# shanjiayao/PTT

Measured on AMD Instinct MI355X. Metric: tracklet frames/sec (hot path: PointNet++ SA stack + Point-Track-Transformer blocks), higher is better.
Workload: dtype f32

## Files before the change

include/ptt_hip.h:

```cpp
#ifndef PTT_HIP_H
#define PTT_HIP_H

#include <stddef.h>
#include <stdint.h>

#ifdef __cplusplus
extern "C" {
#endif

#define PTT_ABI_VERSION 39

enum {
    PTT_OK = 0,
    PTT_EINVAL = -1,
    PTT_EUNSUPPORTED = -2,
    PTT_ELAUNCH = -3,
    PTT_EWORKSPACE = -4
};

typedef void* ptt_stream_t;

int ptt_version(void);
const char* ptt_error_name(int code);
const char* ptt_last_error_string(void);

int ptt_fps_f32(const float* xyz, int B, int N, int npoint, int32_t* idx_out,
                ptt_stream_t stream);
int ptt_fps_ws_f32(const float* xyz, int B, int N, int npoint, int32_t* idx_out, float* workspace,
                   size_t workspace_elems, ptt_stream_t stream);

int ptt_ffps_f32(const float* xyz, const float* feat, int64_t feat_sb, int64_t feat_sc, int64_t feat_sn,
                 int B, int N, int C, int npoint, int32_t* idx_out, ptt_stream_t stream);

int ptt_gather_f32(const float* feat, const int32_t* idx, int B, int C, int N, int M,
                   float* out, ptt_stream_t stream);
int ptt_gather_grad_f32(const float* grad_out, const int32_t* idx, int B, int C, int N,
                        int M, float* grad_feat, ptt_stream_t stream);

int ptt_select_centres_f32(const float* xyz, const int32_t* idx, int B, int N, int M, float* new_xyz,
                           int64_t* idx64_out, ptt_stream_t stream);

int ptt_ball_query_f32(const float* new_xyz, const float* xyz, int B, int M, int N,
                       float radius, int nsample, int32_t* idx_out, ptt_stream_t stream);

int ptt_centres_ball_query_f32(const float* xyz, const int32_t* sel, int B, int N, int M, float radius, int nsample,
                               float* new_xyz, int64_t* idx64_out, int32_t* idx_out, ptt_stream_t stream);

int ptt_group_f32(const float* feat, const int32_t* idx, int B, int C, int N, int M,
                  int ns, float* out, ptt_stream_t stream);
int ptt_group_grad_f32(const float* grad_out, const int32_t* idx, int B, int C, int N,
                       int M, int ns, float* grad_feat, ptt_stream_t stream);

size_t ptt_scatter_add_det_workspace(int B, int N, int E);
int ptt_scatter_add_det_f32(const float* src, const int32_t* idx, int B, int C, int N, int E, float* out,
                            void* workspace, size_t workspace_bytes, ptt_stream_t stream);

int ptt_knn_f32(const float* xyz, int B, int N, int k, int32_t* idx_out,
                ptt_stream_t stream);
int ptt_knn_rel_f32(const float* xyz, int B, int N, int k, int32_t* idx_out, float* rel_out,
                    ptt_stream_t stream);

size_t ptt_packed_weight_elems(int Cout, int K);
int ptt_pack_weight_f32(const float* W, int Cout, int K, float* packed,
                        ptt_stream_t stream);
int ptt_pack_weight_rot_f32(const float* W, int Cout, int K, int rot, float* packed,
                            ptt_stream_t stream);

int ptt_linear_f32(const float* X, int rows, int K, int ldx, const float* Wpacked, int Cout,
                   const float* scale, const float* shift, int relu, const float* residual,
                   int ldr, float* out, int ldo, ptt_stream_t stream);

#define PTT_SA_MAX_LAYERS 4

typedef struct ptt_sa_layer {
    const float* Wpacked;
    const float* scale;
    const float* shift;
    int Cin;
    int Cout;
    int relu;
} ptt_sa_layer;

int ptt_rows_mlp_f32(const float* X, int rows, int K, int ldx, const ptt_sa_layer* layers, int n_layers,
                     const float* residual, int ldr, float* out, int ldo, ptt_stream_t stream);

size_t ptt_ball_query_grid_workspace(int B, int N);
int ptt_ball_query_grid_f32(const float* new_xyz, const float* xyz, int B, int M, int N, float radius, int nsample,
                            int32_t* idx_out, void* workspace, size_t workspace_bytes, ptt_stream_t stream);
int ptt_centres_ball_query_grid_f32(const float* xyz, const int32_t* sel, int B, int N, int M, float radius, int nsample,
                                    float* new_xyz, int64_t* idx64_out, int32_t* idx_out, void* workspace, size_t workspace_bytes,
                                    ptt_stream_t stream);
int ptt_fps_ball_knn_f32(const float* xyz, int B, int N, int M, float radius, int nsample, int k, int32_t* inds,
                         int64_t* inds64, float* new_xyz, int32_t* idx, int32_t* knn, float* rel, ptt_stream_t stream);
// ... 254 lines not shown
#define PTT_REF_CAMERA 0
#define PTT_REF_LIDAR 1
int ptt_box_overlap_f64(const double* gt, const double* pred, int n, int ref_coord, int dims, double* overlap, double* accuracy,
                        ptt_stream_t stream);

#define PTT_TRAIN_MAX_CANDS 1024
typedef struct ptt_train_cand {
    const float* search;
    const uint8_t* label;
    const float* first;
    const float* prev;
    const int32_t* counts;
    float reg[4];
    uint32_t index;
    uint32_t epoch;
    int32_t capacity;
    int32_t reserved;
} ptt_train_cand;

typedef struct ptt_train_batch_desc {
    float* search_points;
    float* template_points;
    float* cls_label;
    float* reg_label;
    int32_t* src_out;
    int32_t* idx_search_out;
    int32_t* idx_template_out;
    int32_t* info;
    int64_t* totals;
    int32_t B, n_cand;
    int32_t search_size, template_size;
    int32_t min_points;
    uint32_t seed_lo, seed_hi;
    int32_t reserved;
} ptt_train_batch_desc;

int ptt_train_batch_f32(const ptt_train_cand* cands_device, const ptt_train_batch_desc* desc_host, ptt_stream_t stream);

typedef struct ptt_train_aug {
    float m[4];
    float kz;
    float reserved[3];
} ptt_train_aug;

int ptt_train_batch_aug_f32(const ptt_train_cand* cands_device, const ptt_train_aug* aug_device, const ptt_train_batch_desc* desc_host,
                            ptt_stream_t stream);
int ptt_philox4x32_10(const uint32_t* counter4, const uint32_t* key2, uint32_t* out4);

size_t ptt_bn_stats_workspace(int R, int C);
int ptt_bn_stats_f32(const float* X, int R, int C, int ldx, float eps, float* mean, float* var, float* invstd,
                     void* workspace, size_t workspace_bytes, ptt_stream_t stream);
int ptt_bn_apply_f32(const float* Z, int ldz, const float* mean, const float* invstd, const float* gamma,
                     const float* beta, int R, int C, int relu, float* X, int ldx, ptt_stream_t stream);
int ptt_bn_bwd_f32(const float* G, int ldg, const float* Act, int lda, const float* Z, int ldz, const float* mean,
                   const float* invstd, const float* gamma, int R, int C, int relu, float* dZ, int ldd,
                   float* dgamma, float* dbeta, void* workspace, size_t workspace_bytes, const float* act_scale,
                   const float* act_shift, ptt_stream_t stream);
int ptt_bn_sums_f64(const float* X, int R, int C, int ldx, double* sums, void* workspace, size_t workspace_bytes,
                    ptt_stream_t stream);
int ptt_bn_finish_f64(const double* sums, int C, float eps, float* mean, float* var, float* invstd,
                      ptt_stream_t stream);
int ptt_bn_bwd_sums_f64(const float* G, int ldg, const float* Act, int lda, const float* Z, int ldz, const float* mean,
                        const float* invstd, int R, int C, double* sums, void* workspace, size_t workspace_bytes,
                        const float* act_scale, const float* act_shift, ptt_stream_t stream);
int ptt_bn_bwd_apply_f32(const float* G, int ldg, const float* Act, int lda, const float* Z, int ldz, const float* mean,
                         const float* invstd, const float* gamma, const float* sum_dy, const float* sum_dy_xhat,
                         const double* count, int R, int C, float* dZ, int ldd, const float* act_scale, const float* act_shift,
                         ptt_stream_t stream);
int ptt_pool_rows_f32(const float* X, int ldx, int G, int ns, int C, float* out, int ldo, int32_t* arg,
                      const float* act_scale, const float* act_shift, ptt_stream_t stream);
int ptt_pool_rows_bwd_f32(const float* dOut, int ldo, const int32_t* arg, int G, int ns, int C, float* dX, int ldx,
                          ptt_stream_t stream);
int ptt_pt_pair_input_f32(const float* q, const float* kf, const int32_t* knn, const float* pos, int B, int N, int k, int D,
                          float* t, ptt_stream_t stream);
int ptt_pt_attn_train_fwd_f32(const float* a, const float* vf, const int32_t* knn, const float* pos, int B, int N, int k, int D,
                              float scale, float* attn, float* res, ptt_stream_t stream);
int ptt_pt_attn_train_bwd_f32(const float* attn, const float* vf, const int32_t* knn, const float* pos, const float* dres, int B,
                              int N, int k, int D, float scale, float* da, float* dvp, ptt_stream_t stream);

int ptt_pt_pair_input_ld_f32(const float* q, int ldq, const float* kf, int ldk, const int32_t* knn, const float* pos, int B, int N,
                             int k, int D, float* t, ptt_stream_t stream);
int ptt_pt_attn_fwd_ld_f32(const float* a, const float* vf, int ldv, const int32_t* knn, const float* pos, int B, int N, int k, int D,
                           float scale, float* attn, float* res, ptt_stream_t stream);

int ptt_gather_rows_f32(const float* src, const int32_t* idx, int B, int N, int E, int C, float* out, ptt_stream_t stream);
int ptt_scatter_csr_i32(const int32_t* idx, int B, int N, int E, int32_t* order, int32_t* start, ptt_stream_t stream);
int ptt_scatter_rows_csr_f32(const float* g, const int32_t* order, const int32_t* start, int B, int N, int E, int C,
                             float* out, ptt_stream_t stream);
int ptt_rows_gemm_pool_supported(int rows, int K, int N, int ldx, int ns);
int ptt_rows_gemm_pool_f32(const float* X, int rows, int K, int ldx, const float* in_scale, const float* in_shift,
                           const float* Wpacked, int N, float* out, int ldo, double* stats, size_t stats_elems, int ns,
                           float* pmax, float* pmin, int32_t* amax, int32_t* amin, ptt_stream_t stream);
int ptt_pool_select_f32(const float* pmax, const float* pmin, const int32_t* amax, const int32_t* amin, const float* act_scale,
                        const float* act_shift, int G, int C, float* out, int32_t* arg, ptt_stream_t stream);
size_t ptt_colsum_workspace(int R, int C);
int ptt_colsum_f32(const float* X, int R, int C, int ldx, float* out, void* workspace, size_t workspace_bytes, ptt_stream_t stream);
size_t ptt_linear_wgrad_workspace(int R, int Cout, int Cin);
int ptt_linear_wgrad_f32(const float* dZ, int ldz, const float* X, int ldx, int R, int Cout, int Cin, float* dW,
                         int accumulate, void* workspace, size_t workspace_bytes, const float* x_scale, const float* x_shift,
                         ptt_stream_t stream);
int ptt_linear_act_in_f32(const float* X, int rows, int K, int ldx, const float* in_scale, const float* in_shift,
                          const float* Wpacked, int Cout, float* out, int ldo, ptt_stream_t stream);

int ptt_pack_weight_strided_f32(const float* W, int Cout, int K, int64_t stride_out, int64_t stride_k, int batch,
                                int64_t stride_batch, float* packed, ptt_stream_t stream);
int ptt_linear_batched_f32(const float* X, int rows, int K, int ldx, int64_t x_batch_stride, const float* Wpacked,
                           int64_t w_batch_stride, int Cout, const float* scale, const float* shift, int relu,
                           const float* residual, int ldr, int64_t r_batch_stride, float* out, int ldo,
                           int64_t o_batch_stride, int batch, ptt_stream_t stream);
int ptt_softmax_rows_f32(float* X, int64_t rows, int n, int ld, float scale, ptt_stream_t stream);
int ptt_layernorm_f32(const float* x, int rows, int C, int ldx, const float* weight, const float* bias, float eps,
                      const float* residual, int ldr, float* out, int ldo, ptt_stream_t stream);

int ptt_rows_gemm_supported(int rows, int K, int N, int ldx, int ldo);
int ptt_rows_gemm_stat_chunks(int rows, int K, int N);
int ptt_rows_gemm_f32(const float* X, int rows, int K, int ldx, const float* in_scale, const float* in_shift,
                      const float* Wpacked, int N, const float* bias, int relu, const float* residual, int ldr,
                      float* out, int ldo, double* stats, size_t stats_elems, ptt_stream_t stream);
int ptt_rows_gemm_masked_f32(const float* X, int rows, int K, int ldx, const float* Wpacked, int N, const float* mask, int ldm,
                             float* out, int ldo, double* stats, size_t stats_elems, ptt_stream_t stream);
int ptt_rows_gemm_bnbwd_f32(const float* X, int rows, int K, int ldx, const float* Wpacked, int N, const float* Z, int ldz,
                            const float* mean, const float* invstd, const float* act_scale, const float* act_shift, float* out,
                            int ldo, double* sums_partial, size_t partial_elems, ptt_stream_t stream);
int ptt_bn_bwd_from_partials_f32(const double* partial, int chunks, const float* G, int ldg, const float* Z, int ldz, const float* mean,
                                 const float* invstd, const float* gamma, int R, int C, float* dZ, int ldd, float* dgamma, float* dbeta,
                                 const float* act_scale, const float* act_shift, ptt_stream_t stream);
int ptt_bn_bwd_sums_partials_f64(const double* partial, int chunks, int C, double* sums, ptt_stream_t stream);
typedef struct ptt_bn_bwd_input {
    const float* g; int ldg;
    const int32_t* arg; int ns;
    const float* z; int ldz;
    const float* k1; const float* c0; const float* c1; const float* mean;
    const float* act_a; const float* act_b;
    float* dz_out; int ldd;
} ptt_bn_bwd_input;
int ptt_bn_bwd_consts_f32(const double* partial, int chunks, const float* mean, const float* invstd, const float* gamma, int R, int C,
                          float* dgamma, float* dbeta, float* k1, float* c0, float* c1, ptt_stream_t stream);
int ptt_bn_bwd_pooled_consts_f32(const float* dPooled, int ldp, const int32_t* arg, int ns, const float* Z, int ldz, const float* mean,
                                 const float* invstd, const float* gamma, int R, int C, float* dgamma, float* dbeta, float* k1,
                                 float* c0, float* c1, void* workspace, size_t workspace_bytes, const float* act_scale,
                                 const float* act_shift, ptt_stream_t stream);
int ptt_rows_gemm_bnbwd_fused_supported(int rows, int K, int N, int ns);
int ptt_rows_gemm_bnbwd_fused_f32(const ptt_bn_bwd_input* in, int rows, int K, const float* Wpacked, int N, const float* Z, int ldz,
                                  const float* mean, const float* invstd, const float* act_scale, const float* act_shift, float* out,
                                  int ldo, double* sums_partial, size_t partial_elems, ptt_stream_t stream);
int ptt_bn_finish_partials_f32(const double* partial, int chunks, int C, int R, float eps, float* mean, float* var, float* invstd,
                               ptt_stream_t stream);
int ptt_bn_sums_partials_f64(const double* partial, int chunks, int C, int R, double* sums, ptt_stream_t stream);
int ptt_bn_bwd_pooled_f32(const float* dPooled, int ldp, const int32_t* arg, int ns, const float* Z, int ldz, const float* mean,
                          const float* invstd, const float* gamma, int R, int C, float* dZ, int ldd, float* dgamma, float* dbeta,
                          void* workspace, size_t workspace_bytes, const float* act_scale, const float* act_shift, ptt_stream_t stream);
int ptt_bn_bwd_pooled_sums_f64(const float* dPooled, int ldp, const int32_t* arg, int ns, const float* Z, int ldz, const float* mean,
                               const float* invstd, int R, int C, double* sums, void* workspace, size_t workspace_bytes,
                               const float* act_scale, const float* act_shift, ptt_stream_t stream);
int ptt_bn_bwd_pooled_apply_f32(const float* dPooled, int ldp, const int32_t* arg, int ns, const float* Z, int ldz, const float* mean,
                                const float* invstd, const float* gamma, const float* sum_dy, const float* sum_dy_xhat,
                                const double* count, int R, int C, float* dZ, int ldd, const float* act_scale,
                                const float* act_shift, ptt_stream_t stream);
int ptt_bn_update_running_f32(const float* mean, const float* var, const double* count, float momentum, int C, float* running_mean,
                              float* running_var, int64_t* num_batches_tracked, ptt_stream_t stream);
int ptt_xcorr_z0_f32(const float* P, const float* cos_t, const float* w_sim, int B, int n2, int n1, int C, float* z0, ptt_stream_t stream);
int ptt_xcorr_z0_stat_chunks(int B, int n2, int n1, int C);
int ptt_xcorr_z0_stats_f32(const float* P, const float* cos_t, const float* w_sim, int B, int n2, int n1, int C, float* z0,
                           double* stats_partial, size_t partial_elems, ptt_stream_t stream);
size_t ptt_xcorr_z0_bwd_workspace(int B, int n1, int C);
int ptt_xcorr_z0_bnbwd_f32(const double* partial, int chunks, const float* G, const float* P, const float* cos_t, const float* w_sim,
// ... 144 lines not shown
```

ptt_amd/build.py:

```python
import os
import shutil
import subprocess
import sys

ROOT = os.path.dirname(os.path.dirname(os.path.abspath(__file__)))
CSRC = os.path.join(ROOT, "ptt_amd", "csrc")
LIBDIR = os.path.join(ROOT, "ptt_amd", "lib")
LIB = os.path.join(LIBDIR, "libptt_hip.so")
HEADER = os.path.join(ROOT, "include", "ptt_hip.h")

HIP_SOURCES = ["errors.hip", "point_ops.hip", "mfma_ops.hip", "track_ops.hip", "train_ops.hip", "gemm_ops.hip", "rowjobs.hip", "step_ops.hip", "wgrad_stream.hip", "pair_split.hip", "sa_split.hip", "xcorr_split.hip"]
EXTRA_FLAGS = {"point_ops.hip": ["-ffp-contract=off"], "track_ops.hip": ["-ffp-contract=off"],
               "mfma_ops.hip": ["-fno-honor-nans"] + os.environ.get("PTT_MFMA_FLAGS", "").split(),
               "gemm_ops.hip": ["-fno-honor-nans"] + os.environ.get("PTT_GEMM_FLAGS", "").split(),
               "rowjobs.hip": ["-fno-honor-nans"],
               "pair_split.hip": ["-fno-honor-nans"],
               "sa_split.hip": ["-fno-honor-nans"],
               "xcorr_split.hip": ["-fno-honor-nans"],
               "wgrad_stream.hip": ["-mllvm", "-amdgpu-mfma-vgpr-form"]}
COMMON_FLAGS = os.environ.get("PTT_HIP_FLAGS", "").split()


def _hipcc():
    return shutil.which("hipcc") or "/opt/rocm/bin/hipcc"


def _stale(target, deps):
    if not os.path.exists(target):
        return True
    t = os.path.getmtime(target)
    return any(os.path.getmtime(d) > t for d in deps)


def build_hip(force=False, verbose=False):
    if force and os.path.isdir(LIBDIR):
        for f in os.listdir(LIBDIR):
            path = os.path.join(LIBDIR, f)
            if os.path.isfile(path):
                os.remove(path)
    os.makedirs(LIBDIR, exist_ok=True)
    headers = [os.path.join(CSRC, f) for f in os.listdir(CSRC) if f.endswith(".h")]
    headers.append(HEADER)
    objs, running = [], []
    for src in HIP_SOURCES:
        s = os.path.join(CSRC, src)
        if not os.path.exists(s):
            continue
        o = os.path.join(LIBDIR, src.replace(".hip", ".o"))
        objs.append(o)
        if force or _stale(o, [s] + headers):
            cmd = [_hipcc(), "--offload-arch=gfx950", "-O3", "-std=c++17", "-fPIC", "-c", s, "-o", o]
            cmd += EXTRA_FLAGS.get(src, []) + COMMON_FLAGS
            if verbose:
                print(" ".join(cmd), flush=True)
            running.append((cmd, subprocess.Popen(cmd)))
    for cmd, proc in running:
        if proc.wait() != 0:
            raise subprocess.CalledProcessError(proc.returncode, cmd)
    if force or _stale(LIB, objs):
        cmd = [_hipcc(), "--offload-arch=gfx950", "-shared", "-fPIC", "-o", LIB] + objs
        if verbose:
            print(" ".join(cmd), flush=True)
        subprocess.check_call(cmd)
    _write_build_id()
    return LIB


def _write_build_id():
    try:
        rev = subprocess.check_output(["git", "rev-parse", "--short", "HEAD"], cwd=ROOT, stderr=subprocess.DEVNULL).decode().strip()
        dirty = subprocess.check_output(["git", "status", "--porcelain", "--", "ptt_amd/csrc", "include"], cwd=ROOT,
                                        stderr=subprocess.DEVNULL).decode().strip()
        with open(os.path.join(LIBDIR, "BUILD_ID"), "w") as fh:
            fh.write("git %s%s\n" % (rev, " + uncommitted kernel changes" if dirty else ""))
    except (OSError, subprocess.CalledProcessError):
        pass


def build_oracle(force=False, verbose=False):
    odir = os.path.join(ROOT, "oracle")
    src = os.path.join(odir, "ptt_oracle.c")
    out = os.path.join(odir, "build", "libptt_oracle.so")
    os.makedirs(os.path.dirname(out), exist_ok=True)
    if force or _stale(out, [src]):
        cmd = ["gcc", "-O2", "-ffp-contract=off", "-fno-fast-math", "-shared", "-fPIC", "-fopenmp", src, "-o", out, "-lm"]
        if verbose:
            print(" ".join(cmd), flush=True)
        subprocess.check_call(cmd)
    return out


if __name__ == "__main__":
    force = "--force" in sys.argv
    print(build_hip(force=force, verbose=True))
    if os.path.exists(os.path.join(ROOT, "oracle", "ptt_oracle.c")):
        print(build_oracle(force=force, verbose=True))
```

ptt_amd/ops.py:

```python
import contextlib
import ctypes
import math
import os

import torch

from . import _lib
from ._lib import AttnDesc, AttnSplitDesc, SaDesc, SaLayer, SaSplitDesc, XcorrDesc, XcorrSplitDesc


def _stream():
    return ctypes.c_void_p(torch.cuda.current_stream().cuda_stream)


_timing = None


def start_kernel_timing(names):
    global _timing
    _timing = {n: [] for n in names}


def stop_kernel_timing():
    global _timing
# ... 1630 lines not shown

def rows_gemm_rsum16_heads(x, wpacked, hd, residual):
    _rows(x, "x"); _rows(residual, "residual")
    rows, D = x.shape
    hd = int(hd)
    if tuple(residual.shape) != (rows, D):
        raise ValueError("rows_gemm_rsum16_heads: residual (rows, D) expected")
    if hd <= 0 or D % hd or wpacked.numel() < hd * hd:
        raise ValueError("rows_gemm_rsum16_heads: D %% hd == 0 and a packed hd x hd weight expected (D=%d hd=%d)" % (D, hd))
    out, plain = (torch.empty((rows, D), dtype=torch.float32, device=x.device) for _ in range(2))
    gsum = torch.empty((rows // 16, D), dtype=torch.float32, device=x.device)
    _launch("ptt_rows_gemm_rsum16_heads_f32", x.device, _ptr(x), rows, D, hd, x.stride(0), _ptr(wpacked), _ptr(residual), residual.stride(0),
            _ptr(out), D, _ptr(plain), D, _ptr(gsum), D, timed='ptt_linear_f32')
    return plain, out, gsum


def layernorm_train_fwd(x, weight, bias, eps, residual=None):
    _rows(x, "x")
    rows, C = x.shape
    for t, name in ((weight, "weight"), (bias, "bias")):
        if t is None or not t.is_cuda or t.dtype != torch.float32 or not t.is_contiguous() or t.numel() != C:
            raise RuntimeError("%s must be a contiguous float32 (%d,) device tensor" % (name, C))
    if residual is not None:
        _rows(residual, "residual")
        if tuple(residual.shape) != (rows, C):
            raise ValueError("layernorm_train_fwd: residual (rows, C) expected")
    y = torch.empty((rows, C), dtype=torch.float32, device=x.device)
    mean, rstd = (torch.empty((rows,), dtype=torch.float32, device=x.device) for _ in range(2))
    _launch("ptt_layernorm_train_fwd_f32", x.device, _ptr(x), rows, C, x.stride(0) if rows > 1 else C, _ptr(weight), _ptr(bias), float(eps),
            _ptr(residual), (residual.stride(0) if (residual is not None and rows > 1) else C), _ptr(y), C, _ptr(mean), _ptr(rstd),
            timed='ptt_layernorm_train_fwd_f32')
    return y, mean, rstd


def layernorm_bwd(dy, x, mean, rstd, weight):
    _rows(dy, "dy"); _rows(x, "x")
    rows, C = x.shape
    if tuple(dy.shape) != (rows, C):
        raise ValueError("layernorm_bwd: dy (rows, C) expected")
    for t, name, n in ((mean, "mean", rows), (rstd, "rstd", rows), (weight, "weight", C)):
        if t is None or not t.is_cuda or t.dtype != torch.float32 or not t.is_contiguous() or t.numel() != n:
            raise RuntimeError("%s must be a contiguous float32 (%d,) device tensor" % (name, n))
    dx = torch.empty((rows, C), dtype=torch.float32, device=x.device)
    dw, db = (torch.empty((C,), dtype=torch.float32, device=x.device) for _ in range(2))
    if rows == 0:
        return dx, dw.zero_(), db.zero_()
    ws, ws_arg = _workspace("ptt_layernorm_bwd_workspace", x.device, rows, C)
    _launch("ptt_layernorm_bwd_f32", x.device, _ptr(dy), dy.stride(0) if rows > 1 else C, _ptr(x), x.stride(0) if rows > 1 else C, _ptr(mean),
            _ptr(rstd), _ptr(weight), rows, C, _ptr(dx), C, _ptr(dw), _ptr(db), *ws_arg, timed='ptt_layernorm_bwd_f32')
    return dx, dw, db


def pt_pair_input(q, kf, knn, pos):
    B, N, D = q.shape
    k = knn.shape[2]
    t = torch.empty((B, N, k, D), dtype=torch.float32, device=q.device)
    _launch("ptt_pt_pair_input_f32", q.device, _ptr(q), _ptr(kf), _ptr(knn), _ptr(pos), B, N, k, D, _ptr(t))
    return t


def pt_pair_input_qkv(qkv, knn, pos, D):
    B, N, _ = qkv.shape
    k = knn.shape[2]
    t = torch.empty((B, N, k, D), dtype=torch.float32, device=qkv.device)
    _launch("ptt_pt_pair_input_ld_f32", qkv.device, qkv.data_ptr(), 3 * D, qkv.data_ptr() + 4 * D, 3 * D, _ptr(knn), _ptr(pos), B, N, k, D, _ptr(t))
    return t


def pt_attn_fwd_qkv(a, qkv, knn, pos, D, scale, want_attn=False):
    B, N, k, _ = a.shape
    res = torch.empty((B, N, D), dtype=torch.float32, device=a.device)
    attn = torch.empty_like(a) if want_attn else None
    _launch("ptt_pt_attn_fwd_ld_f32", a.device, _ptr(a), qkv.data_ptr() + 8 * D, 3 * D, _ptr(knn), _ptr(pos), B, N, k, D, float(scale), _ptr(attn),
            _ptr(res))
    return res, attn


def pt_attn_train_fwd(a, vf, knn, pos, scale):
    B, N, k, D = a.shape
    attn = torch.empty_like(a)
    res = torch.empty((B, N, D), dtype=torch.float32, device=a.device)
    _launch("ptt_pt_attn_train_fwd_f32", a.device, _ptr(a), _ptr(vf), _ptr(knn), _ptr(pos), B, N, k, D, float(scale), _ptr(attn), _ptr(res))
    return attn, res


def pt_attn_train_bwd(attn, vf, knn, pos, dres, scale):
    B, N, k, D = attn.shape
    da, dvp = torch.empty_like(attn), torch.empty_like(attn)
    _launch("ptt_pt_attn_train_bwd_f32", attn.device, _ptr(attn), _ptr(vf), _ptr(knn), _ptr(pos), _ptr(dres), B, N, k, D, float(scale), _ptr(da),
            _ptr(dvp))
    return da, dvp


def _rows2(t, name):
    if t is None:
        return None
    if not t.is_cuda or t.dtype != torch.float32:
        raise RuntimeError("%s must be a float32 device tensor" % name)
    t2 = t.reshape(-1, t.shape[-1])
    if t2.shape[1] > 1 and t2.stride(1) != 1:
        raise RuntimeError("%s must have unit column stride" % name)
    return t2


def _ld(t2):
    return int(t2.stride(0)) if t2.shape[0] > 1 else max(int(t2.shape[1]), int(t2.stride(0)))


def row_job(wpacked, cout, x=None, x2=None, xmax=None, scale=None, shift=None, act=0, res=None, res2=None, res_split=0, out=None,
            out2=None, out_split=0, out_col0=0, raw=None, rel=None, w1=None, qkv=None, knn=None, pos=None, q_off=0,
            k_off=0, v_off=0, N=0, sm_scale=1.0, prologue=0, epilogue=0, K=None, col_tiles=0, idx=None, xyz=None, centres=None,
            wx=None, radius=1.0, ns=0, M=0, normalize_xyz=False, pro_relu=False):
    j = _lib.RowJob()
    keep = [wpacked, scale, shift]
    j.Wpacked, j.scale, j.shift = wpacked.data_ptr(), (scale.data_ptr() if scale is not None else None), \
        (shift.data_ptr() if shift is not None else None)
    j.Cout, j.act, j.prologue, j.epilogue, j.col_tiles = int(cout), int(act), int(prologue), int(epilogue), int(col_tiles)
    if prologue == 0:
        x_ = _rows2(x, "x")
        j.X, j.ldx, j.K1, j.rows = x_.data_ptr(), _ld(x_), x_.shape[1], x_.shape[0]
        j.K = j.K1
        if x2 is not None:
            y_ = _rows2(x2, "x2")
            if y_.shape[0] != x_.shape[0]:
                raise RuntimeError("x and x2 must have the same number of rows")
            j.X2, j.ldx2, j.K = y_.data_ptr(), _ld(y_), j.K1 + y_.shape[1]
            keep.append(y_)
        if xmax is not None:
            m_ = _rows2(xmax, "xmax")
            if m_.shape != x_.shape or _ld(m_) != _ld(x_):
                raise RuntimeError("xmax must have x's shape and row stride")
            j.Xmax = m_.data_ptr()
            keep.append(m_)
        keep.append(x_)
    elif prologue == 1:
        r_ = _rows2(rel, "rel")
        if r_.shape[1] != 3 or not r_.is_contiguous() or w1.shape != (int(K), 4) or not w1.is_contiguous():
            raise RuntimeError("prologue 1: rel (rows,3) and w1 (K,4) contiguous")
        j.rel, j.w1, j.rows, j.K, j.K1 = r_.data_ptr(), w1.data_ptr(), r_.shape[0], int(K), int(K)
        keep += [r_, w1]
    elif prologue == 2:
        j.rows, j.K, j.K1 = pos.reshape(-1, pos.shape[-1]).shape[0], int(K), int(K)
    elif prologue == 3:
        x_ = _rows2(x, "x (per-point term)")
        if (idx.dtype != torch.int32 or not idx.is_contiguous() or not xyz.is_contiguous() or not centres.is_contiguous()
                or not wx.is_contiguous() or tuple(wx.shape) != (3, x_.shape[1])):
            raise RuntimeError("prologue 3: idx int32, xyz / centres / wx (3,K) contiguous")
        j.X, j.ldx, j.K, j.K1, j.rows = x_.data_ptr(), _ld(x_), x_.shape[1], x_.shape[1], idx.numel()
        j.idx, j.xyz, j.centres, j.wx = idx.data_ptr(), xyz.data_ptr(), centres.data_ptr(), wx.data_ptr()
        j.radius, j.normalize_xyz, j.pro_relu, j.N = float(radius), int(bool(normalize_xyz)), int(bool(pro_relu)), int(N)
        keep += [x_, idx, xyz, centres, wx]
    j.ns, j.M = int(ns), int(M)
    if prologue == 2 or epilogue == 1:
        q_, p_ = _rows2(qkv, "qkv"), _rows2(pos, "pos")
        if knn.dtype != torch.int32 or not knn.is_contiguous() or knn.shape[-1] != 16:
            raise RuntimeError("knn must be a contiguous (points,16) int32 tensor")
        j.qkv, j.ldq, j.knn, j.pos, j.ldp = q_.data_ptr(), _ld(q_), knn.data_ptr(), p_.data_ptr(), _ld(p_)
        j.q_off, j.k_off, j.v_off, j.N, j.sm_scale = int(q_off), int(k_off), int(v_off), int(N), float(sm_scale)
        keep += [q_, p_, knn]
    o_ = _rows2(out, "out")
    j.out, j.ldo, j.out_split, j.out_col0 = o_.data_ptr(), _ld(o_), int(out_split), int(out_col0)
    keep.append(o_)
    if out2 is not None:
        o2 = _rows2(out2, "out2")
        j.out2, j.ldo2 = o2.data_ptr(), _ld(o2)
        keep.append(o2)
# ... 302 lines not shown
```

ptt_amd/train_ops.py:

```python
import os
import weakref
from collections import namedtuple

import torch
import torch.distributed as dist
import torch.nn as nn

from . import ops


def _raw_pointer_ready(conv, bn, device):
    ts = [conv.weight] + ([conv.bias] if conv.bias is not None else [])
    if bn is not None:
        ts += [bn.weight, bn.bias, bn.running_mean, bn.running_var]
        nbt = bn.num_batches_tracked
        if nbt is not None and (nbt.dtype != torch.int64 or nbt.device != device):
            return False
    return all(t is not None and t.dtype == torch.float32 and t.device == device and t.is_contiguous() for t in ts)


def _pointwise_conv(conv, conv_cls, one):
    return (isinstance(conv, conv_cls) and conv.kernel_size == one and conv.stride == one and conv.padding == (0,) * len(one)
            and conv.groups == 1)

# ... 627 lines not shown
    wsim, wrest = _SplitCols.apply(w0, 1)
    P = _RowsLinear.apply(rows_i, wrest, None, None)
    return rows_mlp_pool(None, mlp, n1, B, n2, preact=True, front=_XcorrFront(P.contiguous(), cos.contiguous(), wsim.reshape(-1).contiguous()))


class _CosMap(torch.autograd.Function):

    @staticmethod
    def forward(ctx, s, t, eps):
        us, ns = ops.unit_rows_eps(s, eps)
        ut, nt = ops.unit_rows_eps(t, eps)
        cos = torch.bmm(us, ut.transpose(1, 2))
        ctx.save_for_backward(us, ns, ut, nt, cos)
        ctx.like = ((tuple(s.shape), tuple(s.stride())), (tuple(t.shape), tuple(t.stride())))
        return cos

    @staticmethod
    def backward(ctx, g):
        us, ns, ut, nt, cos = ctx.saved_tensors
        g = g.contiguous()
        ds = dt = None
        if ctx.needs_input_grad[0]:
            ds = ops.cos_bwd_rows(torch.bmm(g, ut), us, ns, g, cos, True, ctx.like[0])
        if ctx.needs_input_grad[1]:
            dt = ops.cos_bwd_rows(torch.bmm(g.transpose(1, 2), us), ut, nt, g, cos, False, ctx.like[1])
        return ds, dt, None


class _KnnRel(torch.autograd.Function):

    @staticmethod
    def forward(ctx, xyz, knn, rel):
        ctx.save_for_backward(knn)
        return rel.clone()

    @staticmethod
    def backward(ctx, g):
        (knn,) = ctx.saved_tensors
        B, N, k, _ = g.shape
        back = ops.scatter_add_det(g.permute(0, 3, 1, 2).reshape(B, 3, N * k).contiguous(), knn.view(B, N * k), N)
        return g.sum(dim=2) - back.transpose(1, 2), None, None


class _PairInput(torch.autograd.Function):

    @staticmethod
    def forward(ctx, q, kf, knn, pos, order=None, start=None):
        ctx.save_for_backward(knn, *((order, start) if order is not None else ()))
        return ops.pt_pair_input(q.contiguous(), kf.contiguous(), knn, pos.contiguous())

    @staticmethod
    def backward(ctx, dt):
        knn, csr = ctx.saved_tensors[0], (tuple(ctx.saved_tensors[1:]) or None)
        B, N, k, D = dt.shape
        dt = dt.contiguous()
        dq = dt.sum(dim=2) if ctx.needs_input_grad[0] else None
        dkf = ops.scatter_rows_det(dt.view(B, N * k, D), knn.view(B, N * k), N, csr).neg_() if ctx.needs_input_grad[1] else None
        return dq, dkf, None, dt, None, None


class _AttnAggregate(torch.autograd.Function):

    @staticmethod
    def forward(ctx, a, vf, knn, pos, scale, order=None, start=None):
        ctx.set_materialize_grads(False)
        a, vf, pos = a.contiguous(), vf.contiguous(), pos.contiguous()
        attn, res = ops.pt_attn_train_fwd(a, vf, knn, pos, scale)
        ctx.save_for_backward(attn, vf, knn, pos, *((order, start) if order is not None else ()))
        ctx.scale = float(scale)
        ctx.mark_non_differentiable(attn)
        return res, attn

    @staticmethod
    def backward(ctx, dres, _dattn):
        attn, vf, knn, pos = ctx.saved_tensors[:4]
        csr = tuple(ctx.saved_tensors[4:]) or None
        B, N, k, D = attn.shape
        da, dvp = ops.pt_attn_train_bwd(attn, vf, knn, pos, dres.contiguous(), ctx.scale)
        dvf = ops.scatter_rows_det(dvp.view(B, N * k, D), knn.view(B, N * k), N, csr) if ctx.needs_input_grad[1] else None
        return da, dvf, None, dvp, None, None, None


ATTN_CORE = os.environ.get("PTT_ATTN_CORE", "1") != "0"


class _AttnCore(torch.autograd.Function):

    @staticmethod
    def forward(ctx, q, kf, vf, knn, pos, W1, b1, W2, b2, scale, order, start, heads=1):
        ctx.set_materialize_grads(False)
        q, kf, vf, pos = q.contiguous(), kf.contiguous(), vf.contiguous(), pos.contiguous()
        t = ops.pt_pair_input(q, kf, knn, pos)
        x2 = t.view(-1, t.shape[-1] // heads)
        h, a = _mlp2_forward(x2, W1, b1, W2, b2)
        a = a.view(*t.shape[:-1], W2.shape[0] * heads)
        attn, res = ops.pt_attn_train_fwd(a, vf, knn, pos, scale)
        ctx.save_for_backward(x2, h, attn, vf, knn, pos, order, start, W1, W2)
        ctx.Ws, ctx.bs, ctx.scale, ctx.heads = (W1, W2), (b1, b2), float(scale), int(heads)
        ctx.mark_non_differentiable(attn)
        return res, attn

    @staticmethod
    def backward(ctx, dres, _dattn):
        x2, h, attn, vf, knn, pos, order, start = ctx.saved_tensors[:8]
        W1, W2 = ctx.Ws
        B, N, k, D = attn.shape
        csr = (order, start)
        dres = dres.contiguous()
        da, dvp = ops.pt_attn_train_bwd(attn, vf, knn, pos, dres, ctx.scale)
        dvf = ops.scatter_rows_det(dvp.view(B, N * k, D), knn.view(B, N * k), N, csr)
        heads = ctx.heads
        dz1, dW1, db1, dW2, db2 = _mlp2_backward(da.view(-1, D // heads), x2, h, W1, ctx.bs[0], W2, ctx.bs[1])
        D1, Din = W1.shape
        if heads == 1 and ops.rows_gemm_rsum16_supported(dz1, D1, Din) and k == 16 and Din == D:
            dt, dpos, dq = ops.rows_gemm_rsum16(dz1, packed(W1, True), Din, dvp.view(-1, D))
            dkf = ops.scatter_rows_det(dt.view(B, N * k, D), knn.view(B, N * k), N, csr, negate=True)
            dq, dpos = dq.view(B, N, D), dpos.view(B, N, k, D)
        elif heads > 1 and k == 16 and Din * heads == D and ops.rows_gemm_rsum16_heads_supported(dz1.view(-1, D), D, Din):
            dt, dpos, dq = ops.rows_gemm_rsum16_heads(dz1.view(-1, D), packed(W1, True), Din, dvp.view(-1, D))
            dkf = ops.scatter_rows_det(dt.view(B, N * k, D), knn.view(B, N * k), N, csr, negate=True)
            dq, dpos = dq.view(B, N, D), dpos.view(B, N, k, D)
        else:
            dt = lin_rows(dz1, W1, transpose=True).view(B, N, k, D)
            dq = dt.sum(dim=2)
            dkf = ops.scatter_rows_det(dt.view(B, N * k, D), knn.view(B, N * k), N, csr).neg_()
            dpos = dt + dvp
        return dq, dkf, dvf, None, dpos, dW1, db1, dW2, db2, None, None, None, None


def attn_core(fc_gamma, q, kf, vf, knn, pos, scale, order, start, heads=1):
    return _AttnCore.apply(q, kf, vf, knn, pos, fc_gamma[0].weight, fc_gamma[0].bias, fc_gamma[2].weight, fc_gamma[2].bias, scale, order, start,
                           int(heads))


def pt_block_usable(block, xyz, features):
    return (block.training and xyz.is_cuda and features.dtype == torch.float32 and block.k in (8, 16, 32) and block.d_model % 4 == 0
            and xyz.shape[1] * block.k <= 16384)


MUL_BLOCK_HEADS = (1, 2, 4, 8)


def mul_block_usable(block, xyz, features):
    return bool(block.training and xyz.is_cuda and features.is_cuda and features.dtype == torch.float32 and xyz.dtype == torch.float32
                and block.heads in MUL_BLOCK_HEADS and ops.mul_block_supported(block.d_model, block.k, block.heads)
                and xyz.shape[1] >= block.k
                and xyz.shape[1] * block.k <= 16384 and all(layer.proj_drop.p == 0 for layer in block.layers))


class _RowsLayerNorm(torch.autograd.Function):

    @staticmethod
    def forward(ctx, x, w, b, eps, residual):
        x2 = x.reshape(-1, x.shape[-1]).contiguous()
        r2 = residual.reshape(-1, x.shape[-1]).contiguous() if residual is not None else None
        wd = w.detach()
        y, mean, rstd = ops.layernorm_train_fwd(x2, wd, b.detach(), eps, r2)
        ctx.save_for_backward(x2, mean, rstd, w)
        ctx.w, ctx.b, ctx.shape = w, b, x.shape
        return y.view(x.shape)

    @staticmethod
    def backward(ctx, dy):
        x2, mean, rstd, _ = ctx.saved_tensors
        dy2 = dy.reshape(-1, dy.shape[-1]).contiguous()
        dx, dw, db = ops.layernorm_bwd(dy2, x2, mean, rstd, ctx.w.detach())
        return (dx.view(ctx.shape) if ctx.needs_input_grad[0] else None, small_grad(ctx.w, dw) if ctx.needs_input_grad[1] else None,
                small_grad(ctx.b, db) if ctx.needs_input_grad[2] else None, None, (dy if ctx.needs_input_grad[4] else None))


def rows_layernorm(norm, x, residual=None):
    return _RowsLayerNorm.apply(x, norm.weight, norm.bias, float(norm.eps), residual)


def lin_rows(x2, W, b=None, relu=False, residual=None, transpose=False):
    cout, K = (W.shape[1], W.shape[0]) if transpose else W.shape
    wp = packed(W, transpose)
    if ops.rows_gemm_supported(x2.shape[0], K, cout, x2.stride(0), cout, x=x2):
        return ops.rows_gemm(x2, wp, cout, bias=b, relu=relu, residual=residual)
# ... 205 lines not shown
```

Baseline: 17350.

## Fuse attention-core training forward into one MFMA kernel

```diff
diff --git a/include/ptt_hip.h b/include/ptt_hip.h
--- a/include/ptt_hip.h
+++ b/include/ptt_hip.h
@@ -8,7 +8,7 @@
 extern "C" {
 #endif
 
-#define PTT_ABI_VERSION 39
+#define PTT_ABI_VERSION 40
 
 enum {
     PTT_OK = 0,
@@ -429,6 +429,12 @@
                              int k, int D, float* t, ptt_stream_t stream);
 int ptt_pt_attn_fwd_ld_f32(const float* a, const float* vf, int ldv, const int32_t* knn, const float* pos, int B, int N, int k, int D,
                            float scale, float* attn, float* res, ptt_stream_t stream);
+
+int ptt_pt_attn_core_train_fwd_supported(int B, int N, int k, int D);
+int ptt_pt_attn_core_train_fwd_f32(const float* q, int ldq, const float* kf, int ldk, const float* vf, int ldv, const int32_t* knn,
+                                   const float* pos, const float* W1packed, const float* b1, const float* W2packed, const float* b2,
+                                   int B, int N, int k, int D, float scale, float* t, float* h, float* attn, float* res,
+                                   ptt_stream_t stream);
 
 int ptt_gather_rows_f32(const float* src, const int32_t* idx, int B, int N, int E, int C, float* out, ptt_stream_t stream);
 int ptt_scatter_csr_i32(const int32_t* idx, int B, int N, int E, int32_t* order, int32_t* start, ptt_stream_t stream);
diff --git a/ptt_amd/build.py b/ptt_amd/build.py
--- a/ptt_amd/build.py
+++ b/ptt_amd/build.py
@@ -9,7 +9,7 @@
 LIB = os.path.join(LIBDIR, "libptt_hip.so")
 HEADER = os.path.join(ROOT, "include", "ptt_hip.h")
 
-HIP_SOURCES = ["errors.hip", "point_ops.hip", "mfma_ops.hip", "track_ops.hip", "train_ops.hip", "gemm_ops.hip", "rowjobs.hip", "step_ops.hip", "wgrad_stream.hip", "pair_split.hip", "sa_split.hip", "xcorr_split.hip"]
+HIP_SOURCES = ["errors.hip", "point_ops.hip", "mfma_ops.hip", "track_ops.hip", "train_ops.hip", "gemm_ops.hip", "rowjobs.hip", "step_ops.hip", "wgrad_stream.hip", "pair_split.hip", "sa_split.hip", "xcorr_split.hip", "attn_core_train.hip"]
 EXTRA_FLAGS = {"point_ops.hip": ["-ffp-contract=off"], "track_ops.hip": ["-ffp-contract=off"],
                "mfma_ops.hip": ["-fno-honor-nans"] + os.environ.get("PTT_MFMA_FLAGS", "").split(),
                "gemm_ops.hip": ["-fno-honor-nans"] + os.environ.get("PTT_GEMM_FLAGS", "").split(),
@@ -17,6 +17,7 @@
                "pair_split.hip": ["-fno-honor-nans"],
                "sa_split.hip": ["-fno-honor-nans"],
                "xcorr_split.hip": ["-fno-honor-nans"],
+               "attn_core_train.hip": ["-fno-honor-nans", "-ffp-contract=off"],
                "wgrad_stream.hip": ["-mllvm", "-amdgpu-mfma-vgpr-form"]}
 COMMON_FLAGS = os.environ.get("PTT_HIP_FLAGS", "").split()
 
diff --git a/ptt_amd/csrc/attn_core_train.hip b/ptt_amd/csrc/attn_core_train.hip
--- /dev/null
+++ b/ptt_amd/csrc/attn_core_train.hip
@@ -0,0 +1,245 @@
+#include <math.h>
+#include "common.h"
+#include "mfma_common.h"
+
+namespace ptt {
+
+struct AttnCoreParams {
+    const float* q; const float* kf; const float* vf; const int32_t* knn; const float* pos;
+    const float* W1p; const float* b1; const float* W2p; const float* b2;
+    float* t; float* h; float* attn; float* res;
+    int N, ldq, ldk, ldv;
+    float scale;
+};
+
+namespace {
+
+typedef unsigned int au32x4 __attribute__((__vector_size__(4 * sizeof(unsigned int))));
+
+__device__ __forceinline__ f32x4 ac_load4(__amdgpu_buffer_rsrc_t r, int voff, int soff) {
+    return __builtin_bit_cast(f32x4, __builtin_amdgcn_raw_buffer_load_b128(r, voff, soff, 0));
+}
+__device__ __forceinline__ void ac_store4(f32x4 v, __amdgpu_buffer_rsrc_t r, int voff) {
+    __builtin_amdgcn_raw_buffer_store_b128(__builtin_bit_cast(au32x4, v), r, voff, 0, 0);
+}
+__device__ __forceinline__ __amdgpu_buffer_rsrc_t ac_rsrc(const void* p, int bytes) {
+    return __builtin_amdgcn_make_buffer_rsrc(const_cast<void*>(p), 0, bytes, 0x00020000);
+}
+
+template <int CT>
+__device__ __forceinline__ void ac_prefetch(const float* Wp, int w, int lane, f32x4 (&pre)[CT]) {
+    const __amdgpu_buffer_rsrc_t wr = weight_rsrc(Wp);
+#pragma unroll
+    for (int u = 0; u < CT; ++u) pre[u] = weight_load(wr, (w * 64 + lane) * 16, u * 4 * 1024);
+}
+
+constexpr __device__ __host__ int ac_mem_row(int s) { return 16 * ((s >> 1) & 1) + 4 * (s >> 2) + 2 * (s & 1); }
+
+#ifndef PTT_AC_PF
+#define PTT_AC_PF 1
+#endif
+#ifdef PTT_AC_NOSB
+#define PTT_AC_SB do { } while (0)
+#else
+#define PTT_AC_SB __builtin_amdgcn_sched_barrier(0)
+#endif
+template <int D, bool GATHER>
+__device__ __forceinline__ void ac_gemm(const float* Xs, const float* Wp, int w, int lane, f32x16 (&acc)[D / 128], const f32x4 (&pre)[D / 128],
+                                        const float* srow, __amdgpu_buffer_rsrc_t rout, int svoff,
+                                        __amdgpu_buffer_rsrc_t rv, const int* nbp, int ldv4, int gvoff, f32x4 (&vp)[16]) {
+    constexpr int CT = D / 128, NT = D / 32, NKB = D / 8, LDK = D + 4, PF = PTT_AC_PF;
+    static_assert(NKB == 64, "16 row slots x 4 K-blocks");
+    const float* arow = Xs + (lane & 31) * LDK + 4 * (lane >> 5);
+    const __amdgpu_buffer_rsrc_t wr = weight_rsrc(Wp);
+    const int wvoff = (w * 64 + lane) * 16;
+    constexpr int wkstep = NT * 1024;
+    f32x4 bq[NKB + PF][CT];
+#pragma unroll
+    for (int u = 0; u < CT; ++u) bq[0][u] = pre[u];
+#pragma unroll
+    for (int k = 1; k < PF; ++k)
+#pragma unroll
+        for (int u = 0; u < CT; ++u) bq[k][u] = weight_load(wr, wvoff, k * wkstep + u * 4 * 1024);
+    f32x4 acur = *reinterpret_cast<const f32x4*>(arow), anxt = acur;
+    f32x4 side = {0.f, 0.f, 0.f, 0.f}, g = side;
+    int nbv = 0;
+#pragma unroll
+    for (int kb = 0; kb < NKB; ++kb) {
+        const int s = kb >> 2, ph = kb & 3;
+        if (kb + PF < NKB) {
+#pragma unroll
+            for (int u = 0; u < CT; ++u) bq[kb + PF][u] = weight_load(wr, wvoff, (kb + PF) * wkstep + u * 4 * 1024);
+        }
+        if (kb + 1 < NKB) anxt = *reinterpret_cast<const f32x4*>(arow + (kb + 1) * 8);
+        if (ph == 0) side = *reinterpret_cast<const f32x4*>(srow + 2 * s * LDK);
+        if (ph == 1) ac_store4(side, rout, svoff + ac_mem_row(s) * D * 4);
+        if constexpr (GATHER) {
+            if (ph == 1 && s > 0) vp[s - 1] += g;
+            if (ph == 1) nbv = nbp[2 * s];
+            if (ph == 2) g = ac_load4(rv, nbv * ldv4 + gvoff, 0);
+        }
+        PTT_AC_SB;
+#pragma unroll
+        for (int j = 0; j < 4; ++j)
+#pragma unroll
+            for (int u = 0; u < CT; ++u) acc[u] = __builtin_amdgcn_mfma_f32_32x32x2f32(acur[j], bq[kb][u][j], acc[u], 0, 0, 0);
+        PTT_AC_SB;
+        acur = anxt;
+    }
+    if constexpr (GATHER) vp[15] += g;
+}
+
+}
+
+template <int D>
+__global__ __launch_bounds__(256, 2) void pt_attn_core_train_kernel(AttnCoreParams p) {
+    static_assert(D == 512, "two rows of 128 channel quads per 256 threads");
+    constexpr int CT = D / 128, LDK = D + 4, KNN = 16;
+    extern __shared__ __attribute__((aligned(16))) float smem[];
+    float* Xs = smem;
+    int* nb = reinterpret_cast<int*>(smem + 32 * LDK);
+    const int tid = threadIdx.x, lane = tid & 63, half = lane >> 5, col = lane & 31;
+    const int w = __builtin_amdgcn_readfirstlane(tid >> 6);
+    const int pt0 = logical_block() * 2;
+    f32x4 pre[CT];
+    ac_prefetch<CT>(p.W1p, w, lane, pre);
+
+    if (tid < 32) {
+        const int pp = (tid >> 2) & 1, j = (tid & 3) + 4 * (tid >> 3);
+        nb[tid] = p.knn[(size_t)(pt0 + pp) * KNN + j];
+    }
+    lds_barrier();
+
+    const int cloud = pt0 / p.N;
+    const __amdgpu_buffer_rsrc_t rk = ac_rsrc(p.kf + (size_t)cloud * p.N * p.ldk, ((p.N - 1) * p.ldk + D) * 4);
+    const __amdgpu_buffer_rsrc_t rv = ac_rsrc(p.vf + (size_t)cloud * p.N * p.ldv, ((p.N - 1) * p.ldv + D) * 4);
+    const size_t tile_off = (size_t)pt0 * KNN * D;
+    constexpr int TILE_BYTES = 32 * D * 4;
+    const __amdgpu_buffer_rsrc_t rpos = ac_rsrc(p.pos + tile_off, TILE_BYTES);
+    const __amdgpu_buffer_rsrc_t rt = ac_rsrc(p.t + tile_off, TILE_BYTES), rh = ac_rsrc(p.h + tile_off, TILE_BYTES);
+    const __amdgpu_buffer_rsrc_t rattn = ac_rsrc(p.attn + tile_off, TILE_BYTES);
+    const int qd = tid & 127, rg = tid >> 7;
+    const int svoff = (rg * D + 4 * qd) * 4;
+    float* srow = Xs + rg * LDK + 4 * qd;
+    const int* nbp = nb + rg;
+    const int cw = w * 32 + col;
+    float* xcol = Xs + 4 * half * LDK + cw;
+
+    f32x4 pos[16];
+    {
+        const f32x4 q0 = *reinterpret_cast<const f32x4*>(p.q + (size_t)pt0 * p.ldq + 4 * qd);
+        const f32x4 q1 = *reinterpret_cast<const f32x4*>(p.q + (size_t)(pt0 + 1) * p.ldq + 4 * qd);
+        f32x4 kv[16];
+#pragma unroll
+        for (int s = 0; s < 16; ++s) {
+            pos[s] = ac_load4(rpos, svoff, ac_mem_row(s) * D * 4);
+            kv[s] = ac_load4(rk, nbp[2 * s] * (p.ldk * 4) + qd * 16, 0);
+        }
+#pragma unroll
+        for (int s = 0; s < 16; ++s) {
+            const f32x4 qv = ((s >> 1) & 1) ? q1 : q0;
+            f32x4 tv;
+#pragma unroll
+            for (int x = 0; x < 4; ++x) tv[x] = (qv[x] - kv[s][x]) + pos[s][x];
+            *reinterpret_cast<f32x4*>(srow + 2 * s * LDK) = tv;
+        }
+    }
+    lds_barrier();
+
+    f32x16 acc[CT];
+    {
+#pragma unroll
+        for (int u = 0; u < CT; ++u)
+#pragma unroll
+            for (int j = 0; j < 16; ++j) acc[u][j] = 0.f;
+        ac_gemm<D, false>(Xs, p.W1p, w, lane, acc, pre, srow, rt, svoff, rv, nbp, 0, 0, pos);
+        ac_prefetch<CT>(p.W2p, w, lane, pre);
+        float bv[CT];
+#pragma unroll
+        for (int u = 0; u < CT; ++u) bv[u] = p.b1[u * 128 + cw];
+        lds_barrier();
+#pragma unroll
+        for (int u = 0; u < CT; ++u)
+#pragma unroll
+            for (int j = 0; j < 16; ++j) {
+                xcol[tile_row(j, 0) * LDK + u * 128] = fmaxf(acc[u][j] + bv[u], 0.f);
+                acc[u][j] = 0.f;
+            }
+        lds_barrier();
+    }
+
+    ac_gemm<D, true>(Xs, p.W2p, w, lane, acc, pre, srow, rh, svoff, rv, nbp, p.ldv * 4, qd * 16, pos);
+    lds_barrier();
+#pragma unroll
+    for (int s = 0; s < 16; ++s) *reinterpret_cast<f32x4*>(srow + 2 * s * LDK) = pos[s];
+    lds_barrier();
+
+    {
+        float* rrow = p.res + (size_t)(pt0 + half) * D + cw;
+        const float scale = p.scale;
+#pragma unroll
+        for (int u = 0; u < CT; ++u) {
+            const float bv = p.b2[u * 128 + cw];
+            float y[16], m = -3.0e38f;
+#pragma unroll
+            for (int j = 0; j < 16; ++j) {
+                y[j] = acc[u][j] + bv;
+                m = fmaxf(m, y[j] * scale);
+            }
+            float sum = 0.f;
+#pragma unroll
+            for (int j = 0; j < 16; ++j) {
+                y[j] = __expf(__builtin_fmaf(scale, y[j], -m));
+                sum += y[j];
+            }
+            const float inv = 1.0f / sum;
+            float o = 0.f;
+#pragma unroll
+            for (int j = 0; j < 16; ++j) {
+                float* cell = xcol + tile_row(j, 0) * LDK + u * 128;
+                const float wgt = y[j] * inv;
+                o = __builtin_fmaf(wgt, *cell, o);
+                *cell = wgt;
+            }
+            rrow[u * 128] = o;
+        }
+    }
+    lds_barrier();
+#pragma unroll
+    for (int s = 0; s < 16; ++s) ac_store4(*reinterpret_cast<const f32x4*>(srow + 2 * s * LDK), rattn, svoff + ac_mem_row(s) * D * 4);
+}
+
+}
+
+using namespace ptt;
+
+extern "C" int ptt_pt_attn_core_train_fwd_supported(int B, int N, int k, int D) {
+    if (B < 0 || N <= 0 || (N & 1) || k != 16 || D != 512) return 0;
+    if ((long long)N * 4 * D * 4 >= 0x7fffffffLL || (long long)B * N * k * D >= (1LL << 29)) return 0;
+    return 1;
+}
+
+extern "C" int ptt_pt_attn_core_train_fwd_f32(const float* q, int ldq, const float* kf, int ldk, const float* vf, int ldv, const int32_t* knn,
+                                              const float* pos, const float* W1packed, const float* b1, const float* W2packed,
+                                              const float* b2, int B, int N, int k, int D, float scale, float* t, float* h, float* attn,
+                                              float* res, ptt_stream_t stream) {
+    if (B < 0 || N <= 0 || k <= 0 || D <= 0) return fail(PTT_EINVAL, "ptt_pt_attn_core_train_fwd_f32: B=%d N=%d k=%d D=%d", B, N, k, D);
+    if (!ptt_pt_attn_core_train_fwd_supported(B, N, k, D))
+        return fail(PTT_EUNSUPPORTED, "ptt_pt_attn_core_train_fwd_f32: B=%d N=%d k=%d D=%d (k = 16, D = 512, N even — a tile holds two points of "
+                                      "one cloud — and B N k D < 2^29 are supported)", B, N, k, D);
+    if (ldq < D || ldk < D || ldv < D || (ldq & 3) || (ldk & 3) || (ldv & 3))
+        return fail(PTT_EINVAL, "ptt_pt_attn_core_train_fwd_f32: ldq=%d ldk=%d ldv=%d (each >= D and a multiple of 4)", ldq, ldk, ldv);
+    if ((long long)N * ldk * 4 >= 0x7fffffffLL || (long long)N * ldv * 4 >= 0x7fffffffLL)
+        return fail(PTT_EUNSUPPORTED, "ptt_pt_attn_core_train_fwd_f32: N=%d ldk=%d ldv=%d: a cloud's k / v rows exceed 2 GiB (32-bit offsets)", N,
+                    ldk, ldv);
+    if (!q || !kf || !vf || !knn || !pos || !W1packed || !b1 || !W2packed || !b2 || !t || !h || !attn || !res)
+        return fail(PTT_EINVAL, "ptt_pt_attn_core_train_fwd_f32: null pointer");
+    if (B == 0) return PTT_OK;
+    AttnCoreParams p;
+    p.q = q; p.kf = kf; p.vf = vf; p.knn = knn; p.pos = pos; p.W1p = W1packed; p.b1 = b1; p.W2p = W2packed; p.b2 = b2;
+    p.t = t; p.h = h; p.attn = attn; p.res = res;
+    p.N = N; p.ldq = ldq; p.ldk = ldk; p.ldv = ldv; p.scale = scale;
+    const int lds = (32 * (D + 4) + 32) * (int)sizeof(float);
+    return launch("pt_attn_core_train_kernel", pt_attn_core_train_kernel<512>, dim3((unsigned)((long long)B * N / 2)), dim3(256), lds,
+                  as_stream(stream), p);
+}
diff --git a/ptt_amd/ops.py b/ptt_amd/ops.py
--- a/ptt_amd/ops.py
+++ b/ptt_amd/ops.py
@@ -1736,6 +1736,28 @@
     res = torch.empty((B, N, D), dtype=torch.float32, device=a.device)
     _launch("ptt_pt_attn_train_fwd_f32", a.device, _ptr(a), _ptr(vf), _ptr(knn), _ptr(pos), B, N, k, D, float(scale), _ptr(attn), _ptr(res))
     return attn, res
+
+
+def pt_attn_core_train_fwd_supported(B, N, k, D):
+    return bool(_host("ptt_pt_attn_core_train_fwd_supported", int(B), int(N), int(k), int(D)))
+
+
+def pt_attn_core_train_fwd(q, kf, vf, knn, pos, w1packed, b1, w2packed, b2, scale):
+    B, N, D = q.shape
+    k = knn.shape[2]
+    for x, name in ((q, "q"), (kf, "kf"), (vf, "vf")):
+        if not x.is_cuda or x.dtype != torch.float32 or tuple(x.shape) != (B, N, D) or x.stride(2) != 1 or x.stride(0) != N * x.stride(1):
+            raise RuntimeError("%s must be a float32 device tensor (B, N, D) with unit channel stride and a uniform row stride" % name)
+    _chk(knn, "knn", torch.int32, 3)
+    _chk(pos, "pos", torch.float32, 4)
+    for x, name in ((b1, "b1"), (b2, "b2")):
+        _chk(x, name, torch.float32, 1)
+    t, h, attn = (torch.empty((B, N, k, D), dtype=torch.float32, device=q.device) for _ in range(3))
+    res = torch.empty((B, N, D), dtype=torch.float32, device=q.device)
+    _launch("ptt_pt_attn_core_train_fwd_f32", q.device, _ptr(q), q.stride(1), _ptr(kf), kf.stride(1), _ptr(vf), vf.stride(1), _ptr(knn), _ptr(pos),
+            _ptr(w1packed), _ptr(b1), _ptr(w2packed), _ptr(b2), B, N, k, D, float(scale), _ptr(t), _ptr(h), _ptr(attn), _ptr(res),
+            timed='ptt_pt_attn_core_train_fwd_f32')
+    return t, h, attn, res
 
 
 def pt_attn_train_bwd(attn, vf, knn, pos, dres, scale):
diff --git a/ptt_amd/train_ops.py b/ptt_amd/train_ops.py
--- a/ptt_amd/train_ops.py
+++ b/ptt_amd/train_ops.py
@@ -733,6 +733,7 @@
 
 
 ATTN_CORE = os.environ.get("PTT_ATTN_CORE", "1") != "0"
+ATTN_CORE_FUSED = os.environ.get("PTT_ATTN_CORE_FUSED", "1") != "0"
 
 
 class _AttnCore(torch.autograd.Function):
@@ -741,11 +742,17 @@
     def forward(ctx, q, kf, vf, knn, pos, W1, b1, W2, b2, scale, order, start, heads=1):
         ctx.set_materialize_grads(False)
         q, kf, vf, pos = q.contiguous(), kf.contiguous(), vf.contiguous(), pos.contiguous()
-        t = ops.pt_pair_input(q, kf, knn, pos)
-        x2 = t.view(-1, t.shape[-1] // heads)
-        h, a = _mlp2_forward(x2, W1, b1, W2, b2)
-        a = a.view(*t.shape[:-1], W2.shape[0] * heads)
-        attn, res = ops.pt_attn_train_fwd(a, vf, knn, pos, scale)
+        B, N, D = q.shape
+        if (ATTN_CORE_FUSED and heads == 1 and tuple(W1.shape) == (D, D) and tuple(W2.shape) == (D, D)
+                and ops.pt_attn_core_train_fwd_supported(B, N, knn.shape[2], D)):
+            t, h, attn, res = ops.pt_attn_core_train_fwd(q, kf, vf, knn, pos, packed(W1), b1.detach(), packed(W2), b2.detach(), scale)
+            x2, h = t.view(-1, D), h.view(-1, D)
+        else:
+            t = ops.pt_pair_input(q, kf, knn, pos)
+            x2 = t.view(-1, t.shape[-1] // heads)
+            h, a = _mlp2_forward(x2, W1, b1, W2, b2)
+            a = a.view(*t.shape[:-1], W2.shape[0] * heads)
+            attn, res = ops.pt_attn_train_fwd(a, vf, knn, pos, scale)
         ctx.save_for_backward(x2, h, attn, vf, knn, pos, order, start, W1, W2)
         ctx.Ws, ctx.bs, ctx.scale, ctx.heads = (W1, W2), (b1, b2), float(scale), int(heads)
         ctx.mark_non_differentiable(attn)
```

After: 17390 (median of 3 runs). About the same (+0.2%).
